# ToKe79/nuts333

Hardware: AMD Instinct MI355X
Metric: delivered_broadcast_lines_per_s (higher is better)
Workload: dtype u8

## Files before the change

### nuts333_amd/device/__init__.py

```python
from __future__ import annotations

import ctypes
import os
import shutil
import subprocess
from dataclasses import dataclass, field
from pathlib import Path

import numpy as np

HERE = Path(__file__).resolve().parent
SOURCE = HERE / "fanout.hip"
LIBRARY = HERE / "_build" / "libnuts_device.so"

TEXT_SIZE = 2000
MAX_WRITES = 16
LISTENER_FIELDS = ("login", "has_room", "same_room", "ignall", "ignshout", "is_sender", "colour")
NUM_COMMANDS = 92
COM_SAY, COM_SHOUT, COM_EMOTE, COM_SEMOTE = 3, 4, 6, 7
COM_TELL, COM_PEMOTE = 5, 8
KERNELS = ("nuts_fanout_measure_broadcast", "nuts_fanout_emit_broadcast",
           "nuts_fanout_measure_batch", "nuts_fanout_emit_batch",
           "nuts_fanout_measure_many", "nuts_fanout_emit_many",
           "nuts_roster_measure", "nuts_roster_emit", "nuts_roster_plan", "nuts_roster_record", "nuts_roster_review",
# ... 484 lines not shown
        lib.nd_roster_fanout.argtypes = [ctypes.c_int, ctypes.c_int, P, ctypes.c_int64, P, P, P, P, P, P, P, P, P, P,
                                         ctypes.POINTER(_RosterTiming)]
        lib.nd_roster_fanout.restype = ctypes.c_int
        lib.nd_roster_plan.argtypes = [ctypes.c_int, ctypes.c_int, P, ctypes.c_int64, P, P, P, P, P, P, P, P, P, P, P,
                                       P, ctypes.POINTER(_RosterTiming)]
        lib.nd_roster_plan.restype = ctypes.c_int
        lib.nd_roster_plan_record.argtypes = lib.nd_roster_plan.argtypes + [P]
        lib.nd_roster_plan_record.restype = ctypes.c_int
        lib.nd_roster_review_rooms.argtypes = [ctypes.c_int, ctypes.c_int]
        lib.nd_roster_review_rooms.restype = ctypes.c_int
        lib.nd_roster_review.argtypes = [ctypes.c_int, ctypes.c_int, P, P, P, P, P, P, P, P, P,
                                         ctypes.POINTER(_RosterTiming)]
        lib.nd_roster_review.restype = ctypes.c_int
        lib.nd_roster_speak.argtypes = [ctypes.c_int, ctypes.c_int, P, ctypes.c_int64, P, P, P, P, P, ctypes.c_int,
                                        ctypes.c_int, P, P, P, P, P, P, P, P, P, P, P, ctypes.POINTER(_RosterTiming)]
        lib.nd_roster_speak.restype = ctypes.c_int
        lib.nd_roster_input.argtypes = [ctypes.c_int, ctypes.c_int, P, ctypes.c_int64, P, P, P, ctypes.c_int,
                                        ctypes.c_int, P, P, P, P, P, P, P, P, P, P, P, P, P, P, P, P, P,
                                        ctypes.POINTER(_RosterTiming)]
        lib.nd_roster_input.restype = ctypes.c_int
        lib.nd_roster_revtell_rings.argtypes = [ctypes.c_int]
        lib.nd_roster_revtell_rings.restype = ctypes.c_int
        lib.nd_roster_revtell.argtypes = lib.nd_roster_review.argtypes
        lib.nd_roster_revtell.restype = ctypes.c_int
        lib.nd_roster_tell.argtypes = [ctypes.c_int, ctypes.c_int, P, ctypes.c_int64, P, P, P, P, P, ctypes.c_int,
                                       P, P, P, P, P, P, P, P, P, P, P, P, ctypes.POINTER(_RosterTiming)]
        lib.nd_roster_tell.restype = ctypes.c_int
        lib.nd_roster_look_rooms.argtypes = [ctypes.c_int, ctypes.c_int]
        lib.nd_roster_look_rooms.restype = ctypes.c_int
        lib.nd_roster_look.argtypes = [ctypes.c_int, ctypes.c_int, P, P, ctypes.c_int] + [P] * 18 + [ctypes.POINTER(_RosterTiming)]
        lib.nd_roster_look.restype = ctypes.c_int
        lib.nd_arena.restype = P
        lib.nd_write_sizes.restype = P
        _LIB = lib
    return _LIB


def _check(rc: int, what: str) -> int:
    if rc < 0:
        raise RuntimeError(f"{what}: {_LIB.nd_last_error().decode(errors='replace')}")
    return rc


def _timing_of(t) -> dict:
    return {name: getattr(t, name) for name, _ in t._fields_}


def device_count() -> int:
    n = _load().nd_device_count()
    if n < 0:
        raise RuntimeError(_LIB.nd_last_error().decode(errors="replace"))
    return n


def _ptr(a: np.ndarray) -> int:
    return a.ctypes.data


def _run(broadcast: bool, text: bytes, offs, lens, rec, rm_is_null=0, force_listen=0, com_num=0) -> Fanout:
    lib = _load()
    n = len(rec)
    admitted = np.zeros(n, dtype=np.uint8)
    out_off = np.zeros(n + 1, dtype=np.int64)
    w_off = np.zeros(n + 1, dtype=np.int32)
    tbuf = np.frombuffer(text, dtype=np.uint8) if text else np.zeros(1, dtype=np.uint8)
    t = _Timing()
    rc = lib.nd_fanout(int(broadcast), _ptr(tbuf), len(text), _ptr(offs) if offs is not None else None, _ptr(lens),
                       _ptr(rec), n, rm_is_null, force_listen, com_num, _ptr(admitted), _ptr(out_off), _ptr(w_off),
                       ctypes.byref(t))
    _check(rc, "device fan-out failed")
    return _result(lib, admitted, out_off, w_off, t)


def _result(lib, admitted, out_off, w_off, t) -> Fanout:
    nbytes, nwrites = int(out_off[-1]), int(w_off[-1])
    arena = np.ctypeslib.as_array(ctypes.cast(lib.nd_arena(), ctypes.POINTER(ctypes.c_uint8)), (max(nbytes, 1),))
    wsz = np.ctypeslib.as_array(ctypes.cast(lib.nd_write_sizes(), ctypes.POINTER(ctypes.c_int32)), (max(nwrites, 1),))
    return Fanout(admitted=admitted.astype(bool), out_offsets=out_off, arena=arena[:nbytes].copy(),
                  write_offsets=w_off.astype(np.int64), write_sizes=wsz[:nwrites].copy(),
                  timing=_timing_of(t))


def transduce_batch(texts, colours) -> Fanout:
    text, offs, lens, rec = _prepare_batch(texts, colours)
    return _run(False, text, offs, lens, rec)
# ... 886 lines not shown
```

### nuts333_amd/device/fanout.hip

```cpp

#include <hip/hip_runtime.h>
#include <hipcub/hipcub.hpp>

#include <algorithm>
#include <chrono>
#include <cstdint>
#include <cstdio>
#include <cstring>

namespace {

constexpr int kOutBuff = 1000;
constexpr int kTextSize = 2000;
constexpr int kNumCols = 21;
constexpr int kMaxWrites = 16;
constexpr int kBlock = 256;

constexpr uint8_t kLogin = 1, kHasRoom = 2, kSameRoom = 4, kIgnall = 8, kIgnshout = 16, kSender = 32, kColour = 64;
constexpr int kComShout = 4, kComSemote = 7;

__constant__ char kColCom[kNumCols][2] = {
    {'R', 'S'}, {'O', 'L'}, {'U', 'L'}, {'L', 'I'}, {'R', 'V'}, {'F', 'K'}, {'F', 'R'}, {'F', 'G'}, {'F', 'Y'}, {'F', 'B'},
    {'F', 'M'}, {'F', 'T'}, {'F', 'W'}, {'B', 'K'}, {'B', 'R'}, {'B', 'G'}, {'B', 'Y'}, {'B', 'B'}, {'B', 'M'}, {'B', 'T'},
    {'B', 'W'},
// ... 79 lines not shown
        } else if (ch == '~') {
            if (k.pos > kOutBuff - 6) k.flush();
            const int c = colcom_at(s, i, len);
            if (c >= 0) {
                if (colour) {
                    k.put(27); k.put('['); k.put((uint8_t)kColArg[c][0]);
                    if (kColArg[c][1]) k.put((uint8_t)kColArg[c][1]);
                    k.put('m');
                }
                i += 3;
            } else {
                k.put('~');
                i++;
            }
        } else {
            k.put(ch);
            i++;
        }
        if (k.pos == kOutBuff) k.flush();
    }
    if (k.pos) k.flush();
    if (colour) {
        k.reset_code();
        k.flush();
    }
}

struct Args {
    const uint8_t* text;
    const int32_t* text_off;
    const int32_t* text_len;
    const uint8_t* rec;
    int n;
    int rm_is_null, force_listen, com_num;
    uint8_t* admitted;
    int64_t* nbytes;
    int32_t* nwrites;
    int64_t* out_off;
    int32_t* w_off;
    int* violations;
    uint8_t* arena;
    int64_t arena_cap;
    int32_t* wsz;
    int64_t wsz_cap;
};

template <bool BROADCAST>
__device__ __forceinline__ bool load_item(const Args& a, int i, const uint8_t*& s, int& len)
{
    if (BROADCAST) {
        __shared__ uint8_t lds[kTextSize];
        len = a.text_len[0];
        for (int j = threadIdx.x; j < len; j += blockDim.x) lds[j] = a.text[j];
        __syncthreads();
        s = lds;
        return i < a.n;
    }
    if (i >= a.n) return false;
    s = a.text + a.text_off[i];
    len = a.text_len[i];
    return true;
}

template <bool BROADCAST>
__device__ void measure(const Args& a)
{
    const int i = blockIdx.x * blockDim.x + threadIdx.x;
    if (i == 0) {
        a.nbytes[a.n] = 0;
        a.nwrites[a.n] = 0;
    }
    const uint8_t* s;
    int len;
    if (!load_item<BROADCAST>(a, i, s, len)) return;
    const uint8_t l = a.rec[i];
    const bool in = !BROADCAST || admits(l, a.rm_is_null, a.force_listen, a.com_num);
    Sink<false> k{nullptr, nullptr, 0, 0};
    if (in) transduce(s, len, (l & kColour) != 0, k);
    if (k.n > 6 * (int64_t)len + 4 || k.writes > kMaxWrites) atomicAdd(a.violations, 1);
    a.admitted[i] = in;
    a.nbytes[i] = k.n;
    a.nwrites[i] = k.writes;
}

template <bool BROADCAST>
__device__ void emit(const Args& a)
{
    const int i = blockIdx.x * blockDim.x + threadIdx.x;
    const uint8_t* s;
    int len;
    if (!load_item<BROADCAST>(a, i, s, len) || !a.admitted[i]) return;
    const int64_t room = a.arena_cap - a.out_off[i], wroom = a.wsz_cap - a.w_off[i];
    const int64_t cap = a.nbytes[i] < room ? a.nbytes[i] : (room > 0 ? room : 0);
    const int wcap = (int)(a.nwrites[i] < wroom ? a.nwrites[i] : (wroom > 0 ? wroom : 0));
    Sink<true> k{a.arena + a.out_off[i], a.wsz + a.w_off[i], cap, wcap};
    transduce(s, len, (a.rec[i] & kColour) != 0, k);
}

constexpr int kVarCap = 6 * (kTextSize - 1) + 4;
constexpr int kGroup = 16;

struct ManyArgs {
    const uint8_t* text;
    const int32_t* text_off;
    const int32_t* text_len;
    const uint8_t* flags;
    const int32_t* com_num;
    const int32_t* item_off;
    const int32_t* tile_off;
    const uint8_t* rec;
    int k, m;
    int* violations;
    uint8_t* admitted;
    int64_t* out_off;
    int32_t* w_off;
    int64_t* nbytes;
    int32_t* nwrites;
    uint8_t* arena;
    int64_t arena_cap;
    int32_t* wsz;
    int64_t wsz_cap;
};

struct Tile {
    int b, lo, hi;
};

__device__ __forceinline__ Tile find_tile(const ManyArgs& a)
{
// ... 238 lines not shown
            const int64_t off = a.out_off[i], woff = a.w_off[i];
            const int64_t room = a.arena_cap - off, wroom = a.wsz_cap - woff;
            int64_t n = in ? a.out_off[i + 1] - off : 0;
            n = n < room ? n : room;
            n = n < cap ? n : cap;
            int64_t nw = in ? a.w_off[i + 1] - woff : 0;
            nw = nw < wroom ? nw : wroom;
            nw = nw < kMaxWrites ? nw : kMaxWrites;
            s_off[threadIdx.x] = off;
            s_n[threadIdx.x] = n > 0 ? n : 0;
            s_woff[threadIdx.x] = (int32_t)woff;
            s_nw[threadIdx.x] = nw > 0 ? (int32_t)nw : 0;
            s_c[threadIdx.x] = (a.slot[j] & kColour) ? 1 : 0;
        }
    }
    const uint8_t* src = a.var + var_at(a.text_off[b], b);
    const int64_t stride = var_stride(len);
    for (int c = 0; c < 2; c++) {
        const int64_t n = a.vn[2 * b + c] < cap ? a.vn[2 * b + c] : cap;
        for (int64_t q = threadIdx.x; q < n; q += kBlock) var[c * kVarCap + q] = src[c * stride + q];
        const int nw = a.vw[2 * b + c] < kMaxWrites ? a.vw[2 * b + c] : kMaxWrites;
        if ((int)threadIdx.x < nw) vwsz[c * kMaxWrites + threadIdx.x] = a.vwsz[(2 * b + c) * kMaxWrites + threadIdx.x];
        if (threadIdx.x == 0) {
            vn[c] = n;
            vw[c] = nw;
        }
    }
    __syncthreads();
    const int count = a.capacity - j0 < kBlock ? a.capacity - j0 : kBlock;
    copy_items(count, var, vwsz, vn, vw, s_off, s_n, s_woff, s_nw, s_c, a.arena, a.wsz);
}

static_assert(2 * kMaxWrites <= kBlock, "roster kernels move a broadcast's chunk sizes with one lane each");

struct PlanArgs {
    const int32_t* room;
    const uint8_t* slot;
    const uint8_t* text;
    const int32_t* text_off;
    const int32_t* text_len;
    const int32_t* rm;
    const int32_t* sender;
    const uint8_t* flags;
    const int32_t* com_num;
    int k, capacity, tiles;
    int words;
    int* violations;
    int64_t* vn;
    int32_t* vw;
    int32_t* vwsz;
    uint64_t* bits;
    uint8_t* var;
};

__device__ void roster_plan(const PlanArgs& a)
{
    const int b = (int)blockIdx.x / a.tiles, tile = (int)blockIdx.x - b * a.tiles;
    const int j = tile * kBlock + (int)threadIdx.x;
    bool in = false;
    if (j < a.capacity) {
        const int rm = a.rm[b];
        const uint8_t l = listener_record(a.room[j], a.slot[j], rm, a.sender[b], j);
        in = admits(l, rm < 0, (a.flags[b] >> 1) & 1, a.com_num[b]);
    }
    const uint64_t word = __ballot(in);
    const int w = j >> 6;
// ... 1141 lines not shown
                a.line_slot[line0 + crank] = j;
            } else {
                atomicAdd(a.violations, 1);
            }
        }
        if (looker && shown) {
            if (srank < mcap && crank < lines) {
                a.members[m0 + srank] = j;
                a.mline[m0 + srank] = line0 + crank;
            } else {
                atomicAdd(a.violations, 1);
            }
        }
    }
    if (looker) {
        if (threadIdx.x == 0) a.nmem[b] = seen < mcap ? seen : mcap;
        return;
    }
    for (int i = cands + (int)threadIdx.x; i < lines; i += kBlock) a.clen[text0 + line0 + i] = -1;
    if (threadIdx.x == 0) a.nline[b] = cands < lines ? cands : lines;
}

static_assert(6 + 6 + kNameLen + 1 + kUserDescLen + 5 + 8 + 1 <= kLineRow, "roster_look: the longest member line fits its slot");
static_assert(6 + 6 + kNameLen + 1 + 32 <= kLineRow, "roster_look: the whole description row may be stored before it is cut");
static_assert(kRoomRow % 4 == 0 && kUserDescRow % 4 == 0 && kRrServ + kServNameLen <= kRoomRec, "roster_look: whole words");
static_assert(look_text_cap(0) >= 13 + kRoomNameLen + 2 && look_text_cap(1) >= kRoomDescLen &&
              look_text_cap(2) >= 14 + kMaxLinks * (5 + kRoomNameLen) + 5 + kServNameLen + 1 + 2 &&
              look_text_cap(3) >= 10 + 28 + 21 + 10 + 27 && look_text_cap(4) >= 15 + kTopicLen + 1,
              "roster_look: every room text fits its slot");
static_assert(kLookTextStride < kTextSize, "nuts_roster_speak_plan: a room text fits its LDS text");

}

extern "C" __global__ void __launch_bounds__(kBlock) nuts_fanout_measure_batch(Args a) { measure<false>(a); }
extern "C" __global__ void __launch_bounds__(kBlock) nuts_fanout_measure_broadcast(Args a) { measure<true>(a); }
extern "C" __global__ void __launch_bounds__(kBlock) nuts_fanout_emit_batch(Args a) { emit<false>(a); }
extern "C" __global__ void __launch_bounds__(kBlock) nuts_fanout_emit_broadcast(Args a) { emit<true>(a); }
extern "C" __global__ void __launch_bounds__(kBlock) nuts_fanout_measure_many(ManyArgs a) { measure_many(a); }
extern "C" __global__ void __launch_bounds__(kBlock) nuts_fanout_emit_many(ManyArgs a) { emit_many(a); }
extern "C" __global__ void __launch_bounds__(kBlock) nuts_roster_measure(RosterArgs a) { roster_measure(a); }
extern "C" __global__ void __launch_bounds__(kBlock) nuts_roster_emit(RosterArgs a) { roster_emit(a); }
extern "C" __global__ void __launch_bounds__(kBlock) nuts_roster_plan(PlanArgs a) { roster_plan(a); }
extern "C" __global__ void __launch_bounds__(kBlock) nuts_roster_record(RecordArgs a) { roster_record<kRevLines>(a); }
extern "C" __global__ void __launch_bounds__(kBlock) nuts_roster_review(ReviewArgs a) { roster_review<kRevLines>(a); }
extern "C" __global__ void __launch_bounds__(kBlock) nuts_roster_speak(SpeakArgs a) { roster_speak(a); }
extern "C" __global__ void __launch_bounds__(kBlock) nuts_roster_speak_plan(SpeakPlanArgs a) { roster_speak_plan(a); }
extern "C" __global__ void __launch_bounds__(kBlock) nuts_roster_parse(ParseArgs a) { roster_parse(a); }
extern "C" __global__ void __launch_bounds__(kBlock) nuts_roster_tell(TellArgs a) { roster_tell(a); }
extern "C" __global__ void __launch_bounds__(kBlock) nuts_roster_record_tell(RecordArgs a) { roster_record<kTellLines>(a); }
extern "C" __global__ void __launch_bounds__(kBlock) nuts_roster_revtell(ReviewArgs a) { roster_review<kTellLines>(a); }
extern "C" __global__ void __launch_bounds__(kBlock) nuts_roster_look(LookArgs a) { roster_look(a); }


namespace {

struct Buffers {
    uint8_t* d_block = nullptr;
    size_t cap_block = 0, cap_host_arena = 0, cap_host_writes = 0;
    uint8_t* h_arena = nullptr;
    int32_t* h_wsz = nullptr;
    hipStream_t stream = nullptr;
    hipEvent_t ev0 = nullptr, ev1 = nullptr;
    bool ready = false;
};
Buffers g;
char g_err[512];

int fail(const char* what, hipError_t e)
{
    snprintf(g_err, sizeof(g_err), "%s: %s", what, hipGetErrorString(e));
    return -1;
}

#define ND_CHECK(call)                                  \
    do {                                                \
        hipError_t e_ = (call);                         \
        if (e_ != hipSuccess) return fail(#call, e_);   \
    } while (0)

template <typename T>
int grow_dev(T** p, size_t* cap, size_t want, const char* what)
{
    if (want <= *cap) return 0;
    if (*p) (void)hipFree(*p);
    *p = nullptr;
    *cap = 0;
    hipError_t e = hipMalloc((void**)p, want * sizeof(T));
    if (e != hipSuccess) return fail(what, e);
    *cap = want;
    return 0;
}

template <typename T>
// ... 90 lines not shown
    float ms = 0.f;
    ND_CHECK(hipEventElapsedTime(&ms, g.ev0, g.ev1));
    if (timing) {
        timing->kernels_us = (double)ms * 1e3;
        timing->end_to_end_us = (t1 - t0) * 1e-3;
    }
    return 0;
}

template <typename T>
int fill_timing(T* timing, double t0, double t1, size_t h2d_bytes, size_t d2h_bytes)
{
    if (fill_timing(timing, t0, t1)) return -1;
    if (timing) {
        timing->h2d_bytes = (int64_t)h2d_bytes;
        timing->d2h_bytes = (int64_t)d2h_bytes;
    }
    return 0;
}

int check_bounds(int violations, const char* what)
{
    if (!violations) return 0;
    snprintf(g_err, sizeof(g_err), "%d %s(s) exceeded the hard output bounds (6*len+4 bytes, %d writes)", violations,
             what, kMaxWrites);
    return -1;
}

int fetch_results(const uint8_t* d, size_t res_at, size_t res_bytes)
{
    ND_CHECK(hipEventRecord(g.ev1, g.stream));
    ND_CHECK(hipMemcpyAsync(gm.res, d + res_at, res_bytes, hipMemcpyDeviceToHost, g.stream));
    ND_CHECK(hipStreamSynchronize(g.stream));
    return 0;
}

size_t layout_many(uintptr_t base, size_t text_bytes, size_t scan_bytes, ManyArgs& a, uint8_t** scan)
{
    Carver take{base};
    const size_t k = (size_t)a.k, m = (size_t)a.m;
    take(a.text, text_bytes);
    take(a.text_off, k);
    take(a.text_len, k);
    take(a.flags, k);
    take(a.com_num, k);
    take(a.item_off, k + 1);
    take(a.tile_off, k + 1);
    take(a.rec, m);
    take(a.violations, 1);
    take(a.admitted, m);
    take(a.out_off, m + 1);
    take(a.w_off, m + 1);
    take(a.nbytes, m + 1);
    take(a.nwrites, m + 1);
    take(a.arena, (size_t)a.arena_cap);
    take(a.wsz, (size_t)a.wsz_cap);
    take(*scan, scan_bytes);
    return take.at;
}

constexpr int kMaxRosters = 64;
constexpr int kMaxCapacity = 65536;
struct Roster {
    bool live = false;
    bool resident = false;
    int capacity = 0;
    int64_t rooms = 0;
    uint8_t* d = nullptr;
    uint8_t* mirror = nullptr;
    size_t cap_d = 0, cap_mirror = 0;
    int review_rooms = 0;
    uint8_t* rings = nullptr;
    uint8_t* speech = nullptr;
    bool revtell = false;
    uint8_t* tell_rings = nullptr;
    uint8_t* afk = nullptr;
    int look_rooms = 0;
    uint8_t* room_table = nullptr;
    uint8_t* udesc = nullptr;
};
Roster g_rosters[kMaxRosters];

struct RingSet {
    uint8_t** p;
    int count, lines;
    size_t revline_at() const { return ((size_t)count * lines * kRevSlot + 255) & ~(size_t)255; }
    size_t bytes() const { return revline_at() + (size_t)count * sizeof(int32_t); }
    int32_t* revline() const { return reinterpret_cast<int32_t*>(*p + revline_at()); }
};
RingSet rings_of(Roster& r, bool tell)
{
    return tell ? RingSet{&r.tell_rings, r.revtell ? r.capacity : 0, kTellLines} : RingSet{&r.rings, r.review_rooms, kRevLines};
// ... 291 lines not shown
    return rocprim::make_transform_iterator(rocprim::make_counting_iterator(0),
                                            ItemCount<int32_t>{a.admitted, a.slot, a.vw, a.capacity, m});
}

Roster* roster_at(int handle)
{
    if (handle < 0 || handle >= kMaxRosters || !g_rosters[handle].live) {
        snprintf(g_err, sizeof(g_err), "no live roster %d", handle);
        return nullptr;
    }
    return &g_rosters[handle];
}

}

extern "C" {

struct nd_timing {
    double kernels_us;
    double end_to_end_us;
};

const char* nd_last_error(void) { return g_err; }

int nd_device_count(void)
{
    int n = 0;
    hipError_t e = hipGetDeviceCount(&n);
    if (e == hipErrorNoDevice) return 0;
    if (e != hipSuccess) return fail("hipGetDeviceCount", e);
    return n;
}

int nd_fanout(int broadcast, const uint8_t* text, int64_t text_bytes, const int32_t* text_off, const int32_t* text_len,
              const uint8_t* rec, int n, int rm_is_null, int force_listen, int com_num, uint8_t* admitted,
              int64_t* out_off, int32_t* w_off, nd_timing* timing)
{
    if (ensure_ready()) return -1;
    if (n < 1) {
        snprintf(g_err, sizeof(g_err), "empty batch");
        return -1;
    }
    const double t0 = now_ns();
    hipStream_t st = g.stream;
    Args a{};
    a.n = n;
    a.rm_is_null = rm_is_null;
    a.force_listen = force_listen;
    a.com_num = com_num;
    a.arena_cap = 4 * (int64_t)n + 6 * text_bytes * (broadcast ? n : 1);
    a.wsz_cap = (int64_t)n * kMaxWrites;
    size_t scan1 = 0, scan2 = 0;
    ND_CHECK(hipcub::DeviceScan::ExclusiveSum(nullptr, scan1, a.nbytes, a.out_off, n + 1, st));
    ND_CHECK(hipcub::DeviceScan::ExclusiveSum(nullptr, scan2, a.nwrites, a.w_off, n + 1, st));
    const size_t scan_bytes = std::max(scan1, scan2);
    uint8_t* scan = nullptr;
    const size_t need = layout(0, (size_t)text_bytes, scan_bytes, a, &scan);
    if (grow_dev(&g.d_block, &g.cap_block, need, "device buffers")) return -1;
    layout((uintptr_t)g.d_block, (size_t)text_bytes, scan_bytes, a, &scan);

    ND_CHECK(hipMemcpyAsync((void*)a.text, text, (size_t)text_bytes, hipMemcpyHostToDevice, st));
    ND_CHECK(hipMemcpyAsync((void*)a.text_len, text_len, (broadcast ? 1 : (size_t)n) * sizeof(int32_t), hipMemcpyHostToDevice, st));
    if (!broadcast) ND_CHECK(hipMemcpyAsync((void*)a.text_off, text_off, (size_t)n * sizeof(int32_t), hipMemcpyHostToDevice, st));
    ND_CHECK(hipMemcpyAsync((void*)a.rec, rec, (size_t)n, hipMemcpyHostToDevice, st));
    ND_CHECK(hipMemsetAsync(a.violations, 0, sizeof(int), st));

    const dim3 grid((unsigned)((n + kBlock - 1) / kBlock)), block(kBlock);
    ND_CHECK(hipEventRecord(g.ev0, st));
    hipLaunchKernelGGL(broadcast ? nuts_fanout_measure_broadcast : nuts_fanout_measure_batch, grid, block, 0, st, a);
    ND_CHECK(hipGetLastError());
    size_t bytes = scan_bytes;
    ND_CHECK(hipcub::DeviceScan::ExclusiveSum(scan, bytes, a.nbytes, a.out_off, n + 1, st));
    bytes = scan_bytes;
    ND_CHECK(hipcub::DeviceScan::ExclusiveSum(scan, bytes, a.nwrites, a.w_off, n + 1, st));
    hipLaunchKernelGGL(broadcast ? nuts_fanout_emit_broadcast : nuts_fanout_emit_batch, grid, block, 0, st, a);
    ND_CHECK(hipGetLastError());
    ND_CHECK(hipEventRecord(g.ev1, st));

    int violations = 0;
    ND_CHECK(hipMemcpyAsync(admitted, a.admitted, (size_t)n, hipMemcpyDeviceToHost, st));
    ND_CHECK(hipMemcpyAsync(out_off, a.out_off, ((size_t)n + 1) * sizeof(int64_t), hipMemcpyDeviceToHost, st));
    ND_CHECK(hipMemcpyAsync(w_off, a.w_off, ((size_t)n + 1) * sizeof(int32_t), hipMemcpyDeviceToHost, st));
    ND_CHECK(hipMemcpyAsync(&violations, a.violations, sizeof(int), hipMemcpyDeviceToHost, st));
    ND_CHECK(hipStreamSynchronize(st));
    if (check_bounds(violations, "item")) return -1;
    if (grow_host(&g.h_arena, &g.cap_host_arena, (size_t)out_off[n] + 1, "pinned arena")) return -1;
    if (grow_host(&g.h_wsz, &g.cap_host_writes, (size_t)w_off[n] + 1, "pinned write sizes")) return -1;
    ND_CHECK(hipMemcpyAsync(g.h_arena, a.arena, (size_t)out_off[n], hipMemcpyDeviceToHost, st));
    ND_CHECK(hipMemcpyAsync(g.h_wsz, a.wsz, (size_t)w_off[n] * sizeof(int32_t), hipMemcpyDeviceToHost, st));
    ND_CHECK(hipStreamSynchronize(st));
    const double t1 = now_ns();

    return fill_timing(timing, t0, t1);
}

const uint8_t* nd_arena(void) { return g.h_arena; }
const int32_t* nd_write_sizes(void) { return g.h_wsz; }

int nd_fanout_many(int k, const uint8_t* text, int64_t text_bytes, const int32_t* text_off, const int32_t* text_len,
                   const uint8_t* flags, const int32_t* com_num, const int32_t* item_off, const uint8_t* rec,
                   uint8_t* admitted, int64_t* out_off, int32_t* w_off, nd_timing* timing)
{
    if (ensure_ready()) return -1;
    if (k < 1 || item_off[0] != 0) {
        snprintf(g_err, sizeof(g_err), "empty call, or item offsets that do not start at 0");
        return -1;
    }
    for (int b = 0; b < k; b++)
        if (item_off[b + 1] <= item_off[b]) {
            snprintf(g_err, sizeof(g_err), "broadcast %d has no listeners", b);
            return -1;
        }
    const double t0 = now_ns();
    hipStream_t st = g.stream;
    ManyArgs a{};
    a.k = k;
    a.m = item_off[k];
    for (int b = 0; b < k; b++) a.arena_cap += (int64_t)(item_off[b + 1] - item_off[b]) * (6 * (int64_t)text_len[b] + 4);
    a.wsz_cap = (int64_t)a.m * kMaxWrites;
    const int m = a.m;
    size_t scan1 = 0, scan2 = 0;
    ND_CHECK(hipcub::DeviceScan::ExclusiveSum(nullptr, scan1, a.nbytes, a.out_off, m + 1, st));
    ND_CHECK(hipcub::DeviceScan::ExclusiveSum(nullptr, scan2, a.nwrites, a.w_off, m + 1, st));
    const size_t scan_bytes = std::max(scan1, scan2);
    uint8_t* scan = nullptr;
    ManyArgs o = a;
    const size_t need = layout_many(0, (size_t)text_bytes, scan_bytes, o, &scan);
    if (grow_dev(&g.d_block, &g.cap_block, need, "device buffers")) return -1;
    layout_many((uintptr_t)g.d_block, (size_t)text_bytes, scan_bytes, a, &scan);
    const size_t in_bytes = (uintptr_t)o.violations + sizeof(int);
// ... 3 lines not shown

    uint8_t* h = gm.stage;
    const Put put{h};
    put(o.text, text, (size_t)text_bytes);
    put(o.text_off, text_off, (size_t)k * sizeof(int32_t));
    put(o.text_len, text_len, (size_t)k * sizeof(int32_t));
    put(o.flags, flags, (size_t)k);
    put(o.com_num, com_num, (size_t)k * sizeof(int32_t));
    put(o.item_off, item_off, ((size_t)k + 1) * sizeof(int32_t));
    int32_t* tiles = reinterpret_cast<int32_t*>(h + (uintptr_t)o.tile_off);
    tiles[0] = 0;
    for (int b = 0; b < k; b++) tiles[b + 1] = tiles[b] + (item_off[b + 1] - item_off[b] + kBlock - 1) / kBlock;
    put(o.rec, rec, (size_t)m);
    *reinterpret_cast<int*>(h + (uintptr_t)o.violations) = 0;
    ND_CHECK(hipMemcpyAsync(g.d_block, h, in_bytes, hipMemcpyHostToDevice, st));

    const dim3 grid((unsigned)tiles[k]), block(kBlock);
    ND_CHECK(hipEventRecord(g.ev0, st));
    hipLaunchKernelGGL(nuts_fanout_measure_many, grid, block, 0, st, a);
    ND_CHECK(hipGetLastError());
    size_t bytes = scan_bytes;
    ND_CHECK(hipcub::DeviceScan::ExclusiveSum(scan, bytes, a.nbytes, a.out_off, m + 1, st));
    bytes = scan_bytes;
    ND_CHECK(hipcub::DeviceScan::ExclusiveSum(scan, bytes, a.nwrites, a.w_off, m + 1, st));
    hipLaunchKernelGGL(nuts_fanout_emit_many, grid, block, 0, st, a);
    ND_CHECK(hipGetLastError());

    if (fetch_results(g.d_block, res_at, res_bytes)) return -1;
    const Res res{gm.res, res_at};
    if (check_bounds(*reinterpret_cast<const int*>(res(o.violations)), "item")) return -1;
    memcpy(admitted, res(o.admitted), (size_t)m);
    memcpy(out_off, res(o.out_off), ((size_t)m + 1) * sizeof(int64_t));
    memcpy(w_off, res(o.w_off), ((size_t)m + 1) * sizeof(int32_t));
    if (grow_host(&g.h_arena, &g.cap_host_arena, (size_t)out_off[m] + 1, "pinned arena")) return -1;
    if (grow_host(&g.h_wsz, &g.cap_host_writes, (size_t)w_off[m] + 1, "pinned write sizes")) return -1;
    ND_CHECK(hipMemcpyAsync(g.h_arena, a.arena, (size_t)out_off[m], hipMemcpyDeviceToHost, st));
    ND_CHECK(hipMemcpyAsync(g.h_wsz, a.wsz, (size_t)w_off[m] * sizeof(int32_t), hipMemcpyDeviceToHost, st));
    ND_CHECK(hipStreamSynchronize(st));
    const double t1 = now_ns();

    return fill_timing(timing, t0, t1);
}

struct nd_roster_timing {
    double kernels_us;
    double end_to_end_us;
    int64_t h2d_bytes;
    int64_t d2h_bytes;
};

int nd_roster_create(int capacity)
{
    if (capacity < 1 || capacity > kMaxCapacity) {
        snprintf(g_err, sizeof(g_err), "roster capacity %d outside 1 .. %d", capacity, kMaxCapacity);
        return -1;
    }
    for (int h = 0; h < kMaxRosters; h++)
        if (!g_rosters[h].live) {
            g_rosters[h] = Roster{};
            g_rosters[h].live = true;
            g_rosters[h].capacity = capacity;
            return h;
        }
    snprintf(g_err, sizeof(g_err), "%d rosters are live: destroy one first", kMaxRosters);
    return -1;
}

int nd_roster_destroy(int handle)
{
    Roster* r = roster_at(handle);
    if (!r) return -1;
// ... 50 lines not shown
    if (grow_host(&gm.res, &gm.cap_res, res_bytes, "pinned results")) return -1;

    uint8_t* h = r->mirror;
    const Put put{h};
    put(o.text, text, (size_t)text_bytes);
    put(o.text_off, text_off, (size_t)k * sizeof(int32_t));
    put(o.text_len, text_len, (size_t)k * sizeof(int32_t));
    put(o.rm, rm, (size_t)k * sizeof(int32_t));
    put(o.sender, sender, (size_t)k * sizeof(int32_t));
    put(o.flags, flags, (size_t)k);
    put(o.com_num, com_num, (size_t)k * sizeof(int32_t));
    *reinterpret_cast<int*>(h + (uintptr_t)o.violations) = 0;
    const size_t from = r->resident ? table_bytes : 0;
    ND_CHECK(hipMemcpyAsync(r->d + from, h + from, in_bytes - from, hipMemcpyHostToDevice, st));
    r->resident = true;

    const dim3 grid((unsigned)(k * a.tiles)), block(kBlock);
    ND_CHECK(hipEventRecord(g.ev0, st));
    hipLaunchKernelGGL(nuts_roster_measure, grid, block, 0, st, a);
    ND_CHECK(hipGetLastError());
    size_t bytes = scan_bytes;
    ND_CHECK(hipcub::DeviceScan::ExclusiveSum(scan, bytes, item_bytes(a, m), a.out_off, m + 1, st));
    bytes = scan_bytes;
    ND_CHECK(hipcub::DeviceScan::ExclusiveSum(scan, bytes, item_writes(a, m), a.w_off, m + 1, st));
    hipLaunchKernelGGL(nuts_roster_emit, grid, block, 0, st, a);
    ND_CHECK(hipGetLastError());

    if (fetch_results(r->d, res_at, res_bytes)) return -1;
    const Res res{gm.res, res_at};
    if (check_bounds(*reinterpret_cast<const int*>(res(o.violations)), "variant")) return -1;
    memcpy(admitted, res(o.admitted), (size_t)m);
    memcpy(out_off, res(o.out_off), ((size_t)m + 1) * sizeof(int64_t));
    memcpy(w_off, res(o.w_off), ((size_t)m + 1) * sizeof(int32_t));
    if (grow_host(&g.h_arena, &g.cap_host_arena, (size_t)out_off[m] + 1, "pinned arena")) return -1;
    if (grow_host(&g.h_wsz, &g.cap_host_writes, (size_t)w_off[m] + 1, "pinned write sizes")) return -1;
    ND_CHECK(hipMemcpyAsync(g.h_arena, a.arena, (size_t)out_off[m], hipMemcpyDeviceToHost, st));
    ND_CHECK(hipMemcpyAsync(g.h_wsz, a.wsz, (size_t)w_off[m] * sizeof(int32_t), hipMemcpyDeviceToHost, st));
    ND_CHECK(hipStreamSynchronize(st));
    const double t1 = now_ns();

    return fill_timing(timing, t0, t1, in_bytes - from,
                       res_bytes + (size_t)out_off[m] + (size_t)w_off[m] * sizeof(int32_t));
}

static int plan_call(int handle, int k, const uint8_t* text, int64_t text_bytes, const int32_t* text_off,
                     const int32_t* text_len, const int32_t* rm, const int32_t* sender, const uint8_t* flags,
                     const int32_t* com_num, const uint8_t* table, uint64_t* bits, int64_t* vn, int32_t* vw,
                     int32_t* vwsz, uint8_t* var, nd_roster_timing* timing, bool record, const uint8_t* clear)
{
    Roster* r = roster_at(handle);
    if (!r || ensure_ready()) return -1;
    if (record && ensure_rings(*r, g.stream)) return -1;
    const int cap = r->capacity, words = (cap + 63) / 64;
    if (k < 1 || (int64_t)k * cap >= INT32_MAX || text_bytes < 0) {
        snprintf(g_err, sizeof(g_err), "%d broadcasts to %d slots: need 1 <= k * capacity < 2^31 - 1", k, cap);
        return -1;
    }
    const double t0 = now_ns();
    hipStream_t st = g.stream;
    PlanArgs a{};
    a.k = k;
    a.capacity = cap;
    a.tiles = (cap + kBlock - 1) / kBlock;
    a.words = words;
    const size_t var_bytes = (size_t)var_at(text_bytes, k);
    PlanArgs o = a;
    const size_t clear_bytes = record && clear ? (size_t)r->review_rooms : 0;
    const uint8_t *o_clear = nullptr, *d_clear = nullptr;
    const size_t need = layout_plan(0, (size_t)text_bytes, var_bytes, o, clear_bytes, &o_clear);
    const size_t table_bytes = (uintptr_t)o.text, in_bytes = (uintptr_t)o.violations + sizeof(int);
    const size_t res_at = (uintptr_t)o.violations, res_bytes = (uintptr_t)o.var + var_bytes - res_at;
// ... 601 lines not shown
```

### nuts333_amd/devpath.py

```python
from __future__ import annotations

import argparse
import ctypes
import json
import statistics
import subprocess
import sys
import time
from pathlib import Path

import numpy as np

from nuts333_amd import device, nuts_path

REPO = Path(__file__).resolve().parent.parent
PATHBENCH = REPO / "oracle" / "_build" / "pathbench"

TEXTS = {
    "say": b"Uaaa says: synthetic broadcast line 000123 from the nuts333 bench\n",
    "shout": b"~OLUaaa shouts:~RS synthetic broadcast line 000123 from the nuts333 bench\n",
}
COM = {"say": device.COM_SAY, "shout": device.COM_SHOUT}
SIZES = (10, 100, 1000)
COLOURS = ("off", "on", "half")
# ... 581 lines not shown
                         for n in SIZES for text in TEXTS for colour in COLOURS for k in a.per_call],
        }
    roster = {}
    if a.roster:
        roster = {
            "roster_kernels": ["nuts_roster_measure", "rocprim device scan x2", "nuts_roster_emit"],
            "roster_end_to_end_covers": "packing the K inputs into pinned memory, one H2D (the roster table only in a "
                                        "call after an update: h2d_bytes_first_call), kernels, three D2H, two "
                                        "synchronises (python_us adds checking the K tuples and the copies out of "
                                        "pinned memory)",
            "roster": [roster_case(n, text, colour, k, a.reps, a.warmup, pb)
                       for n in SIZES for text in TEXTS for colour in COLOURS for k in a.roster],
        }
    plan = {}
    if a.plan:
        plan = {
            "plan_kernels": ["nuts_roster_plan"],
            "plan_end_to_end_covers": "packing the K inputs into pinned memory, one H2D (the roster table only in a "
                                      "call after an update: h2d_bytes_first_call), one kernel, one D2H of the "
                                      "variants, their chunk sizes and the admit bitmap at their bound size, one "
                                      "synchronise (python_us adds checking the K tuples, the copies out of pinned "
                                      "memory and building the Plan; expand() is not timed)",
            "plan": [plan_case(n, text, colour, k, a.reps, a.warmup, pb)
                     for n in SIZES for text in TEXTS for colour in COLOURS for k in a.plan],
        }
    review = review_cases(a.review, a.reps, a.warmup, pb) if a.review else {}
    speak = speak_cases(a.speak, a.reps, a.warmup, pb) if a.speak else {}
    inputs = input_cases(a.input, a.reps, a.warmup, pb) if a.input else {}
    tell = tell_cases(a.tell, a.reps, a.warmup, pb) if a.tell else {}
    look = look_cases(a.look, a.reps, a.warmup, pb) if a.look else {}
    out = {
        "what": "user-space stage of one broadcast (admit predicate + transducer), device vs CPU",
        "device": "gfx950",
        "kernels": ["nuts_fanout_measure_broadcast", "rocprim device scan x2", "nuts_fanout_emit_broadcast"],
        "reps": a.reps, "warmup": a.warmup,
        "end_to_end_covers": "listener table + text H2D, kernels, admitted/offsets/arena/write-size D2H, synchronise",
        "cpu_derived_from": {"pathbench": {k: v for k, v in pb.items() if k not in ("sink", "admitted")},
                             "formula": "(N-1) x transduce + N x fanout_predicate + format_line_once (derived, not timed)"},
        "cases": cases,
        **per_call,
        **roster,
        **plan,
        **review,
        **speak,
        **inputs,
        **tell,
        **look,
        "wall_s": round(time.perf_counter() - t_start, 1),
    }
    print(json.dumps(out))
    return 0


if __name__ == "__main__":
    sys.exit(main())
```

Measured before the change: 751,000.

## Compute broadcast variants once and lay out listeners by count instead of scanning

The broadcast path used to run the transducer once per listener, then two device scans for offsets, then emit per listener. It now renders the colour-off and colour-on variants once, counts admitted listeners per tile with wave ballots, and derives each listener's offsets from those counts in the emit kernel, which copies the shared variant bytes. Inputs go up in a single packed pinned H2D and results come back in a single D2H when they fit under a 1 MiB limit, cutting launch and copy count. The cost is a host-side bound computation and a per-tile prefix loop over earlier tiles' counts, which grows with the number of tiles.

```diff
diff --git a/nuts333_amd/device/__init__.py b/nuts333_amd/device/__init__.py
--- a/nuts333_amd/device/__init__.py
+++ b/nuts333_amd/device/__init__.py
@@ -540,6 +540,12 @@
         lib.nd_roster_look.restype = ctypes.c_int
         lib.nd_arena.restype = P
         lib.nd_write_sizes.restype = P
+        lib.nd_broadcast_bound.argtypes = [ctypes.c_char_p, ctypes.c_int, ctypes.POINTER(ctypes.c_int64),
+                                           ctypes.POINTER(ctypes.c_int32)]
+        lib.nd_broadcast_bound.restype = None
+        lib.nd_single_fetch_limit.restype = ctypes.c_int64
+        lib.nd_broadcast_result_bytes.argtypes = [ctypes.c_char_p, ctypes.c_int, ctypes.c_int]
+        lib.nd_broadcast_result_bytes.restype = ctypes.c_int64
         _LIB = lib
     return _LIB
 
@@ -559,6 +565,20 @@
     if n < 0:
         raise RuntimeError(_LIB.nd_last_error().decode(errors="replace"))
     return n
+
+
+def broadcast_bound(text: bytes) -> tuple[int, int]:
+    nbytes, nwrites = ctypes.c_int64(), ctypes.c_int32()
+    _load().nd_broadcast_bound(text, len(text), ctypes.byref(nbytes), ctypes.byref(nwrites))
+    return nbytes.value, nwrites.value
+
+
+def broadcast_result_bytes(text: bytes, n: int) -> int:
+    return int(_load().nd_broadcast_result_bytes(text, len(text), n))
+
+
+def single_fetch_limit() -> int:
+    return int(_load().nd_single_fetch_limit())
 
 
 def _ptr(a: np.ndarray) -> int:
diff --git a/nuts333_amd/device/fanout.hip b/nuts333_amd/device/fanout.hip
--- a/nuts333_amd/device/fanout.hip
+++ b/nuts333_amd/device/fanout.hip
@@ -135,7 +135,6 @@
     const int32_t* text_len;
     const uint8_t* rec;
     int n;
-    int rm_is_null, force_listen, com_num;
     uint8_t* admitted;
     int64_t* nbytes;
     int32_t* nwrites;
@@ -148,24 +147,6 @@
     int64_t wsz_cap;
 };
 
-template <bool BROADCAST>
-__device__ __forceinline__ bool load_item(const Args& a, int i, const uint8_t*& s, int& len)
-{
-    if (BROADCAST) {
-        __shared__ uint8_t lds[kTextSize];
-        len = a.text_len[0];
-        for (int j = threadIdx.x; j < len; j += blockDim.x) lds[j] = a.text[j];
-        __syncthreads();
-        s = lds;
-        return i < a.n;
-    }
-    if (i >= a.n) return false;
-    s = a.text + a.text_off[i];
-    len = a.text_len[i];
-    return true;
-}
-
-template <bool BROADCAST>
 __device__ void measure(const Args& a)
 {
     const int i = blockIdx.x * blockDim.x + threadIdx.x;
@@ -173,31 +154,25 @@
         a.nbytes[a.n] = 0;
         a.nwrites[a.n] = 0;
     }
-    const uint8_t* s;
-    int len;
-    if (!load_item<BROADCAST>(a, i, s, len)) return;
-    const uint8_t l = a.rec[i];
-    const bool in = !BROADCAST || admits(l, a.rm_is_null, a.force_listen, a.com_num);
+    if (i >= a.n) return;
+    const int len = a.text_len[i];
     Sink<false> k{nullptr, nullptr, 0, 0};
-    if (in) transduce(s, len, (l & kColour) != 0, k);
+    transduce(a.text + a.text_off[i], len, (a.rec[i] & kColour) != 0, k);
     if (k.n > 6 * (int64_t)len + 4 || k.writes > kMaxWrites) atomicAdd(a.violations, 1);
-    a.admitted[i] = in;
+    a.admitted[i] = true;
     a.nbytes[i] = k.n;
     a.nwrites[i] = k.writes;
 }
 
-template <bool BROADCAST>
 __device__ void emit(const Args& a)
 {
     const int i = blockIdx.x * blockDim.x + threadIdx.x;
-    const uint8_t* s;
-    int len;
-    if (!load_item<BROADCAST>(a, i, s, len) || !a.admitted[i]) return;
+    if (i >= a.n) return;
     const int64_t room = a.arena_cap - a.out_off[i], wroom = a.wsz_cap - a.w_off[i];
     const int64_t cap = a.nbytes[i] < room ? a.nbytes[i] : (room > 0 ? room : 0);
     const int wcap = (int)(a.nwrites[i] < wroom ? a.nwrites[i] : (wroom > 0 ? wroom : 0));
     Sink<true> k{a.arena + a.out_off[i], a.wsz + a.w_off[i], cap, wcap};
-    transduce(s, len, (a.rec[i] & kColour) != 0, k);
+    transduce(a.text + a.text_off[i], a.text_len[i], (a.rec[i] & kColour) != 0, k);
 }
 
 constexpr int kVarCap = 6 * (kTextSize - 1) + 4;
@@ -502,6 +477,141 @@
 }
 
 static_assert(2 * kMaxWrites <= kBlock, "roster kernels move a broadcast's chunk sizes with one lane each");
+
+struct BcastArgs {
+    const uint8_t* text;
+    const int32_t* text_off;
+    const int32_t* text_len;
+    const uint8_t* rec;
+    int n;
+    int rm_is_null, force_listen, com_num;
+    int* violations;
+    uint8_t* admitted;
+    int64_t* out_off;
+    int32_t* w_off;
+    int32_t* tile_count;
+    uint8_t* var;
+    int64_t* vn;
+    int32_t* vw;
+    int32_t* vwsz;
+    uint8_t* arena;
+    int64_t arena_cap;
+    int32_t* wsz;
+    int64_t wsz_cap;
+};
+
+constexpr int kWaves = kBlock / 64;
+
+__device__ void measure_broadcast(const BcastArgs& a)
+{
+    __shared__ int s_count[2][kWaves];
+    const int i = (int)blockIdx.x * kBlock + (int)threadIdx.x;
+    bool in = false, on = false;
+    if (i < a.n) {
+        const uint8_t l = a.rec[i];
+        in = admits(l, a.rm_is_null, a.force_listen, a.com_num);
+        on = (l & kColour) != 0;
+        a.admitted[i] = in;
+    }
+    const uint64_t m_off = __ballot(in && !on), m_on = __ballot(in && on);
+    if ((threadIdx.x & 63) == 0) {
+        s_count[0][threadIdx.x >> 6] = __popcll(m_off);
+        s_count[1][threadIdx.x >> 6] = __popcll(m_on);
+    }
+    __syncthreads();
+    if (threadIdx.x < 2) {
+        int sum = 0;
+        for (int w = 0; w < kWaves; w++) sum += s_count[threadIdx.x][w];
+        a.tile_count[2 * blockIdx.x + threadIdx.x] = sum;
+    }
+    if (blockIdx.x == 0) store_variants(a, 0);
+}
+
+__device__ void emit_broadcast(const BcastArgs& a)
+{
+    __shared__ uint8_t var[2 * kVarCap];
+    __shared__ int32_t vwsz[2 * kMaxWrites];
+    __shared__ int64_t vn[2];
+    __shared__ int vw[2];
+    __shared__ int64_t s_off[kBlock], s_n[kBlock];
+    __shared__ int32_t s_woff[kBlock], s_nw[kBlock];
+    __shared__ uint8_t s_c[kBlock];
+    __shared__ int s_before[2][kWaves], s_count[2][kWaves];
+    const int tile = (int)blockIdx.x, lane = (int)threadIdx.x & 63, wave = (int)threadIdx.x >> 6;
+    const int len = a.text_len[0];
+    const int64_t cap = 6 * (int64_t)len + 4;
+    const int64_t bytes_off = a.vn[0], bytes_on = a.vn[1];
+    const int writes_off = a.vw[0], writes_on = a.vw[1];
+    int b_off = 0, b_on = 0;
+    for (int t = (int)threadIdx.x; t < tile; t += kBlock) {
+        b_off += a.tile_count[2 * t];
+        b_on += a.tile_count[2 * t + 1];
+    }
+    for (int d = 32; d; d >>= 1) {
+        b_off += __shfl_xor(b_off, d);
+        b_on += __shfl_xor(b_on, d);
+    }
+    const int i = tile * kBlock + (int)threadIdx.x;
+    bool in = false, on = false;
+    if (i < a.n) {
+        in = a.admitted[i] != 0;
+        on = (a.rec[i] & kColour) != 0;
+    }
+    const uint64_t m_off = __ballot(in && !on), m_on = __ballot(in && on);
+    if (lane == 0) {
+        s_before[0][wave] = b_off;
+        s_before[1][wave] = b_on;
+        s_count[0][wave] = __popcll(m_off);
+        s_count[1][wave] = __popcll(m_on);
+    }
+    __syncthreads();
+    const uint64_t below = ((uint64_t)1 << lane) - 1;
+    int64_t c_off = __popcll(m_off & below), c_on = __popcll(m_on & below);
+    for (int w = 0; w < kWaves; w++) {
+        c_off += s_before[0][w] + (w < wave ? s_count[0][w] : 0);
+        c_on += s_before[1][w] + (w < wave ? s_count[1][w] : 0);
+    }
+    const int64_t off = c_off * bytes_off + c_on * bytes_on, woff = c_off * writes_off + c_on * writes_on;
+    if (i < a.n) {
+        a.out_off[i] = off;
+        a.w_off[i] = (int32_t)woff;
+        const int64_t room = a.arena_cap - off, wroom = a.wsz_cap - woff;
+        int64_t n = in ? (on ? bytes_on : bytes_off) : 0;
+        n = n < room ? n : room;
+        n = n < cap ? n : cap;
+        int64_t nw = in ? (on ? writes_on : writes_off) : 0;
+        nw = nw < wroom ? nw : wroom;
+        nw = nw < kMaxWrites ? nw : kMaxWrites;
+        s_off[threadIdx.x] = off;
+        s_n[threadIdx.x] = n > 0 ? n : 0;
+        s_woff[threadIdx.x] = (int32_t)woff;
+        s_nw[threadIdx.x] = nw > 0 ? (int32_t)nw : 0;
+        s_c[threadIdx.x] = on ? 1 : 0;
+    }
+    if (tile == (int)gridDim.x - 1 && threadIdx.x == kBlock - 1) {
+        const int64_t total = off + (in ? (on ? bytes_on : bytes_off) : 0);
+        const int64_t wtotal = woff + (in ? (on ? writes_on : writes_off) : 0);
+        a.out_off[a.n] = total;
+        a.w_off[a.n] = (int32_t)wtotal;
+        if (total > a.arena_cap || wtotal > a.wsz_cap) atomicAdd(a.violations, 1);
+    }
+    const int64_t stride = var_stride(len);
+    for (int c = 0; c < 2; c++) {
+        const int64_t vb = c ? bytes_on : bytes_off, n = vb < cap ? vb : cap;
+        for (int64_t q = threadIdx.x; q < n; q += kBlock) var[c * kVarCap + q] = a.var[c * stride + q];
+        const int vc = c ? writes_on : writes_off, nw = vc < kMaxWrites ? vc : kMaxWrites;
+        if ((int)threadIdx.x < nw) vwsz[c * kMaxWrites + threadIdx.x] = a.vwsz[c * kMaxWrites + threadIdx.x];
+        if (threadIdx.x == 0) {
+            vn[c] = n;
+            vw[c] = nw;
+        }
+    }
+    __syncthreads();
+    const int count = a.n - tile * kBlock < kBlock ? a.n - tile * kBlock : kBlock;
+    copy_items(count, var, vwsz, vn, vw, s_off, s_n, s_woff, s_nw, s_c, a.arena, a.wsz);
+}
+
+static_assert(kBlock % 64 == 0, "the broadcast kernels count a tile's items a wave at a time");
 
 struct PlanArgs {
     const int32_t* room;
@@ -1709,10 +1819,10 @@
 
 }
 
-extern "C" __global__ void __launch_bounds__(kBlock) nuts_fanout_measure_batch(Args a) { measure<false>(a); }
-extern "C" __global__ void __launch_bounds__(kBlock) nuts_fanout_measure_broadcast(Args a) { measure<true>(a); }
-extern "C" __global__ void __launch_bounds__(kBlock) nuts_fanout_emit_batch(Args a) { emit<false>(a); }
-extern "C" __global__ void __launch_bounds__(kBlock) nuts_fanout_emit_broadcast(Args a) { emit<true>(a); }
+extern "C" __global__ void __launch_bounds__(kBlock) nuts_fanout_measure_batch(Args a) { measure(a); }
+extern "C" __global__ void __launch_bounds__(kBlock) nuts_fanout_measure_broadcast(BcastArgs a) { measure_broadcast(a); }
+extern "C" __global__ void __launch_bounds__(kBlock) nuts_fanout_emit_batch(Args a) { emit(a); }
+extern "C" __global__ void __launch_bounds__(kBlock) nuts_fanout_emit_broadcast(BcastArgs a) { emit_broadcast(a); }
 extern "C" __global__ void __launch_bounds__(kBlock) nuts_fanout_measure_many(ManyArgs a) { measure_many(a); }
 extern "C" __global__ void __launch_bounds__(kBlock) nuts_fanout_emit_many(ManyArgs a) { emit_many(a); }
 extern "C" __global__ void __launch_bounds__(kBlock) nuts_roster_measure(RosterArgs a) { roster_measure(a); }
@@ -1736,6 +1846,8 @@
     size_t cap_block = 0, cap_host_arena = 0, cap_host_writes = 0;
     uint8_t* h_arena = nullptr;
     int32_t* h_wsz = nullptr;
+    const uint8_t* out_arena = nullptr;
+    const int32_t* out_wsz = nullptr;
     hipStream_t stream = nullptr;
     hipEvent_t ev0 = nullptr, ev1 = nullptr;
     bool ready = false;
@@ -1892,6 +2004,18 @@
     ND_CHECK(hipEventRecord(g.ev1, g.stream));
     ND_CHECK(hipMemcpyAsync(gm.res, d + res_at, res_bytes, hipMemcpyDeviceToHost, g.stream));
     ND_CHECK(hipStreamSynchronize(g.stream));
+    return 0;
+}
+
+int fetch_arena(const uint8_t* arena, size_t nbytes, const int32_t* wsz, size_t nwrites)
+{
+    if (grow_host(&g.h_arena, &g.cap_host_arena, nbytes + 1, "pinned arena")) return -1;
+    if (grow_host(&g.h_wsz, &g.cap_host_writes, nwrites + 1, "pinned write sizes")) return -1;
+    ND_CHECK(hipMemcpyAsync(g.h_arena, arena, nbytes, hipMemcpyDeviceToHost, g.stream));
+    ND_CHECK(hipMemcpyAsync(g.h_wsz, wsz, nwrites * sizeof(int32_t), hipMemcpyDeviceToHost, g.stream));
+    ND_CHECK(hipStreamSynchronize(g.stream));
+    g.out_arena = g.h_arena;
+    g.out_wsz = g.h_wsz;
     return 0;
 }
 
@@ -1918,6 +2042,30 @@
     take(*scan, scan_bytes);
     return take.at;
 }
+
+size_t layout_bcast(uintptr_t base, size_t text_bytes, BcastArgs& a)
+{
+    Carver take{base};
+    const size_t n = (size_t)a.n, tiles = (n + kBlock - 1) / kBlock;
+    take(a.text, text_bytes);
+    take(a.text_off, 1);
+    take(a.text_len, 1);
+    take(a.rec, n);
+    take(a.violations, 1);
+    take(a.admitted, n);
+    take(a.out_off, n + 1);
+    take(a.w_off, n + 1);
+    take(a.wsz, (size_t)a.wsz_cap);
+    take(a.arena, (size_t)a.arena_cap);
+    take(a.tile_count, 2 * tiles);
+    take(a.var, (size_t)var_at((int64_t)text_bytes, 1));
+    take(a.vn, 2);
+    take(a.vw, 2);
+    take(a.vwsz, 2 * kMaxWrites);
+    return take.at;
+}
+
+constexpr size_t kSingleFetchLimit = (size_t)1 << 20;
 
 constexpr int kMaxRosters = 64;
 constexpr int kMaxCapacity = 65536;
@@ -2275,6 +2423,95 @@
     return n;
 }
 
+void nd_broadcast_bound(const uint8_t* text, int len, int64_t* bytes, int32_t* writes)
+{
+    int64_t newlines = 0, tildes = 0;
+    for (int i = 0; i < len; i++) {
+        newlines += text[i] == '\n';
+        tildes += text[i] == '~';
+    }
+    const int64_t b = std::min(len + 5 * newlines + 2 * tildes + 4, 6 * (int64_t)len + 4);
+    *bytes = b;
+    *writes = (int32_t)std::min(b / (kOutBuff - 5) + 2, (int64_t)kMaxWrites);
+}
+
+static size_t bcast_offsets(const uint8_t* text, int len, int n, BcastArgs& o)
+{
+    int64_t item_bytes = 0;
+    int32_t item_writes = 0;
+    nd_broadcast_bound(text, len, &item_bytes, &item_writes);
+    o.n = n;
+    o.arena_cap = n * item_bytes;
+    o.wsz_cap = (int64_t)n * item_writes;
+    return layout_bcast(0, (size_t)len, o);
+}
+
+int64_t nd_broadcast_result_bytes(const uint8_t* text, int len, int n)
+{
+    BcastArgs o{};
+    bcast_offsets(text, len, n, o);
+    return (int64_t)((uintptr_t)o.arena + (size_t)o.arena_cap - (uintptr_t)o.violations);
+}
+int64_t nd_single_fetch_limit(void) { return (int64_t)kSingleFetchLimit; }
+
+static int fanout_broadcast(const uint8_t* text, int len, const uint8_t* rec, int n, int rm_is_null, int force_listen,
+                            int com_num, uint8_t* admitted, int64_t* out_off, int32_t* w_off, nd_timing* timing)
+{
+    const double t0 = now_ns();
+    hipStream_t st = g.stream;
+    BcastArgs o{};
+    const size_t need = bcast_offsets(text, len, n, o);
+    if (grow_dev(&g.d_block, &g.cap_block, need, "device buffers")) return -1;
+    BcastArgs a = o;
+    a.rm_is_null = rm_is_null;
+    a.force_listen = force_listen;
+    a.com_num = com_num;
+    layout_bcast((uintptr_t)g.d_block, (size_t)len, a);
+    const size_t res_at = (uintptr_t)o.violations, in_bytes = res_at + sizeof(int);
+    const size_t all_bytes = (uintptr_t)o.arena + (size_t)o.arena_cap - res_at;
+    const bool single = all_bytes <= kSingleFetchLimit;
+    const size_t res_bytes = single ? all_bytes : (uintptr_t)o.wsz - res_at;
+    if (grow_host(&gm.stage, &gm.cap_stage, in_bytes, "pinned staging")) return -1;
+    if (grow_host(&gm.res, &gm.cap_res, res_bytes, "pinned results")) return -1;
+
+    uint8_t* h = gm.stage;
+    const Put put{h};
+    put(o.text, text, (size_t)len);
+    *reinterpret_cast<int32_t*>(h + (uintptr_t)o.text_off) = 0;
+    *reinterpret_cast<int32_t*>(h + (uintptr_t)o.text_len) = len;
+    put(o.rec, rec, (size_t)n);
+    *reinterpret_cast<int*>(h + (uintptr_t)o.violations) = 0;
+    ND_CHECK(hipMemcpyAsync(g.d_block, h, in_bytes, hipMemcpyHostToDevice, st));
+
+    const dim3 grid((unsigned)((n + kBlock - 1) / kBlock)), block(kBlock);
+    ND_CHECK(hipEventRecord(g.ev0, st));
+    hipLaunchKernelGGL(nuts_fanout_measure_broadcast, grid, block, 0, st, a);
+    ND_CHECK(hipGetLastError());
+    hipLaunchKernelGGL(nuts_fanout_emit_broadcast, grid, block, 0, st, a);
+    ND_CHECK(hipGetLastError());
+
+    if (fetch_results(g.d_block, res_at, res_bytes)) return -1;
+    const Res res{gm.res, res_at};
+    if (*reinterpret_cast<const int*>(res(o.violations))) {
+        snprintf(g_err, sizeof(g_err), "a variant exceeded the hard output bounds (6*len+4 bytes, %d writes), or the %d items "
+                 "the capacities nd_broadcast_bound gives (%lld bytes, %lld writes)", kMaxWrites, n, (long long)o.arena_cap,
+                 (long long)o.wsz_cap);
+        return -1;
+    }
+    memcpy(admitted, res(o.admitted), (size_t)n);
+    memcpy(out_off, res(o.out_off), ((size_t)n + 1) * sizeof(int64_t));
+    memcpy(w_off, res(o.w_off), ((size_t)n + 1) * sizeof(int32_t));
+    if (single) {
+        g.out_arena = res(o.arena);
+        g.out_wsz = reinterpret_cast<const int32_t*>(res(o.wsz));
+    } else if (fetch_arena(a.arena, (size_t)out_off[n], a.wsz, (size_t)w_off[n])) {
+        return -1;
+    }
+    const double t1 = now_ns();
+
+    return fill_timing(timing, t0, t1);
+}
+
 int nd_fanout(int broadcast, const uint8_t* text, int64_t text_bytes, const int32_t* text_off, const int32_t* text_len,
               const uint8_t* rec, int n, int rm_is_null, int force_listen, int com_num, uint8_t* admitted,
               int64_t* out_off, int32_t* w_off, nd_timing* timing)
@@ -2284,14 +2521,13 @@
         snprintf(g_err, sizeof(g_err), "empty batch");
         return -1;
     }
+    if (broadcast)
+        return fanout_broadcast(text, text_len[0], rec, n, rm_is_null, force_listen, com_num, admitted, out_off, w_off, timing);
     const double t0 = now_ns();
     hipStream_t st = g.stream;
     Args a{};
     a.n = n;
-    a.rm_is_null = rm_is_null;
-    a.force_listen = force_listen;
-    a.com_num = com_num;
-    a.arena_cap = 4 * (int64_t)n + 6 * text_bytes * (broadcast ? n : 1);
+    a.arena_cap = 4 * (int64_t)n + 6 * text_bytes;
     a.wsz_cap = (int64_t)n * kMaxWrites;
     size_t scan1 = 0, scan2 = 0;
     ND_CHECK(hipcub::DeviceScan::ExclusiveSum(nullptr, scan1, a.nbytes, a.out_off, n + 1, st));
@@ -2303,20 +2539,20 @@
     layout((uintptr_t)g.d_block, (size_t)text_bytes, scan_bytes, a, &scan);
 
     ND_CHECK(hipMemcpyAsync((void*)a.text, text, (size_t)text_bytes, hipMemcpyHostToDevice, st));
-    ND_CHECK(hipMemcpyAsync((void*)a.text_len, text_len, (broadcast ? 1 : (size_t)n) * sizeof(int32_t), hipMemcpyHostToDevice, st));
-    if (!broadcast) ND_CHECK(hipMemcpyAsync((void*)a.text_off, text_off, (size_t)n * sizeof(int32_t), hipMemcpyHostToDevice, st));
+    ND_CHECK(hipMemcpyAsync((void*)a.text_len, text_len, (size_t)n * sizeof(int32_t), hipMemcpyHostToDevice, st));
+    ND_CHECK(hipMemcpyAsync((void*)a.text_off, text_off, (size_t)n * sizeof(int32_t), hipMemcpyHostToDevice, st));
     ND_CHECK(hipMemcpyAsync((void*)a.rec, rec, (size_t)n, hipMemcpyHostToDevice, st));
     ND_CHECK(hipMemsetAsync(a.violations, 0, sizeof(int), st));
 
     const dim3 grid((unsigned)((n + kBlock - 1) / kBlock)), block(kBlock);
     ND_CHECK(hipEventRecord(g.ev0, st));
-    hipLaunchKernelGGL(broadcast ? nuts_fanout_measure_broadcast : nuts_fanout_measure_batch, grid, block, 0, st, a);
+    hipLaunchKernelGGL(nuts_fanout_measure_batch, grid, block, 0, st, a);
     ND_CHECK(hipGetLastError());
     size_t bytes = scan_bytes;
     ND_CHECK(hipcub::DeviceScan::ExclusiveSum(scan, bytes, a.nbytes, a.out_off, n + 1, st));
     bytes = scan_bytes;
     ND_CHECK(hipcub::DeviceScan::ExclusiveSum(scan, bytes, a.nwrites, a.w_off, n + 1, st));
-    hipLaunchKernelGGL(broadcast ? nuts_fanout_emit_broadcast : nuts_fanout_emit_batch, grid, block, 0, st, a);
+    hipLaunchKernelGGL(nuts_fanout_emit_batch, grid, block, 0, st, a);
     ND_CHECK(hipGetLastError());
     ND_CHECK(hipEventRecord(g.ev1, st));
 
@@ -2327,18 +2563,14 @@
     ND_CHECK(hipMemcpyAsync(&violations, a.violations, sizeof(int), hipMemcpyDeviceToHost, st));
     ND_CHECK(hipStreamSynchronize(st));
     if (check_bounds(violations, "item")) return -1;
-    if (grow_host(&g.h_arena, &g.cap_host_arena, (size_t)out_off[n] + 1, "pinned arena")) return -1;
-    if (grow_host(&g.h_wsz, &g.cap_host_writes, (size_t)w_off[n] + 1, "pinned write sizes")) return -1;
-    ND_CHECK(hipMemcpyAsync(g.h_arena, a.arena, (size_t)out_off[n], hipMemcpyDeviceToHost, st));
-    ND_CHECK(hipMemcpyAsync(g.h_wsz, a.wsz, (size_t)w_off[n] * sizeof(int32_t), hipMemcpyDeviceToHost, st));
-    ND_CHECK(hipStreamSynchronize(st));
+    if (fetch_arena(a.arena, (size_t)out_off[n], a.wsz, (size_t)w_off[n])) return -1;
     const double t1 = now_ns();
 
     return fill_timing(timing, t0, t1);
 }
 
-const uint8_t* nd_arena(void) { return g.h_arena; }
-const int32_t* nd_write_sizes(void) { return g.h_wsz; }
+const uint8_t* nd_arena(void) { return g.out_arena; }
+const int32_t* nd_write_sizes(void) { return g.out_wsz; }
 
 int nd_fanout_many(int k, const uint8_t* text, int64_t text_bytes, const int32_t* text_off, const int32_t* text_len,
                    const uint8_t* flags, const int32_t* com_num, const int32_t* item_off, const uint8_t* rec,
@@ -2408,11 +2640,7 @@
     memcpy(admitted, res(o.admitted), (size_t)m);
     memcpy(out_off, res(o.out_off), ((size_t)m + 1) * sizeof(int64_t));
     memcpy(w_off, res(o.w_off), ((size_t)m + 1) * sizeof(int32_t));
-    if (grow_host(&g.h_arena, &g.cap_host_arena, (size_t)out_off[m] + 1, "pinned arena")) return -1;
-    if (grow_host(&g.h_wsz, &g.cap_host_writes, (size_t)w_off[m] + 1, "pinned write sizes")) return -1;
-    ND_CHECK(hipMemcpyAsync(g.h_arena, a.arena, (size_t)out_off[m], hipMemcpyDeviceToHost, st));
-    ND_CHECK(hipMemcpyAsync(g.h_wsz, a.wsz, (size_t)w_off[m] * sizeof(int32_t), hipMemcpyDeviceToHost, st));
-    ND_CHECK(hipStreamSynchronize(st));
+    if (fetch_arena(a.arena, (size_t)out_off[m], a.wsz, (size_t)w_off[m])) return -1;
     const double t1 = now_ns();
 
     return fill_timing(timing, t0, t1);
@@ -2529,11 +2757,7 @@
     memcpy(admitted, res(o.admitted), (size_t)m);
     memcpy(out_off, res(o.out_off), ((size_t)m + 1) * sizeof(int64_t));
     memcpy(w_off, res(o.w_off), ((size_t)m + 1) * sizeof(int32_t));
-    if (grow_host(&g.h_arena, &g.cap_host_arena, (size_t)out_off[m] + 1, "pinned arena")) return -1;
-    if (grow_host(&g.h_wsz, &g.cap_host_writes, (size_t)w_off[m] + 1, "pinned write sizes")) return -1;
-    ND_CHECK(hipMemcpyAsync(g.h_arena, a.arena, (size_t)out_off[m], hipMemcpyDeviceToHost, st));
-    ND_CHECK(hipMemcpyAsync(g.h_wsz, a.wsz, (size_t)w_off[m] * sizeof(int32_t), hipMemcpyDeviceToHost, st));
-    ND_CHECK(hipStreamSynchronize(st));
+    if (fetch_arena(a.arena, (size_t)out_off[m], a.wsz, (size_t)w_off[m])) return -1;
     const double t1 = now_ns();
 
     return fill_timing(timing, t0, t1, in_bytes - from,
diff --git a/nuts333_amd/devpath.py b/nuts333_amd/devpath.py
--- a/nuts333_amd/devpath.py
+++ b/nuts333_amd/devpath.py
@@ -637,9 +637,10 @@
     out = {
         "what": "user-space stage of one broadcast (admit predicate + transducer), device vs CPU",
         "device": "gfx950",
-        "kernels": ["nuts_fanout_measure_broadcast", "rocprim device scan x2", "nuts_fanout_emit_broadcast"],
+        "kernels": ["nuts_fanout_measure_broadcast", "nuts_fanout_emit_broadcast"],
         "reps": a.reps, "warmup": a.warmup,
-        "end_to_end_covers": "listener table + text H2D, kernels, admitted/offsets/arena/write-size D2H, synchronise",
+        "end_to_end_covers": "packing the text and the listener records into pinned memory, one H2D, two kernels, one D2H "
+                             "of admitted/offsets/write sizes/arena at their bound size, one synchronise",
         "cpu_derived_from": {"pathbench": {k: v for k, v in pb.items() if k not in ("sink", "admitted")},
                              "formula": "(N-1) x transduce + N x fanout_predicate + format_line_once (derived, not timed)"},
         "cases": cases,
```

Measured after the change: 745,800. Within noise of the previous version (-0.7%).
